# Mistra-UEA/Mistra

Hardware: AMD Instinct MI355X
Metric: chemistry-timesteps/sec (tot mechanism) (higher is better)
Workload: dtype f64; 1 GPU; tot mechanism, 100000 synthetic cells per GPU (100000 total), INTEGRATE_t(0,10 s), Ros3 rtol 1e-3; perturbed captured BTZ96 cloud states; cells_per_gpu=100000, failed_cells=0, parallelism=cells sharded over 1 GPU(s), no data-path collective

## Files before the change

### mistra_amd/build.py

```python
import os
import shutil
import subprocess
import sys

PKG = os.path.dirname(os.path.abspath(__file__))
CSRC = os.path.join(PKG, "csrc")
LIBDIR = os.path.join(PKG, "lib")
OBJDIR = os.path.join(PKG, "build")
LIB = os.path.join(LIBDIR, "libmistra_chem.so")

ARCH = "gfx950"
COMMON = ["-O3", "-std=c++17", "-fPIC", "-ffp-contract=off", "-fno-fast-math", "-Wall", "-Wno-unused-function"]
SOURCES = ["mech_tables.cpp", "schedule.cpp", "capi.cpp", "ros3_kernel.hip", "rates.hip", "pack.hip"]


def hipcc():
    for cand in (os.environ.get("HIPCC"), shutil.which("hipcc"), "/opt/rocm/bin/hipcc"):
        if cand and os.path.exists(cand):
            return cand
    raise RuntimeError("hipcc not found")


def _stale(target, deps):
    if not os.path.exists(target):
# ... 31 lines not shown
            print(" ".join(cmd))
        subprocess.run(cmd, check=True)
    return LIB


def ring_register_report(isa_path=None):
    import re
    import tempfile
    with tempfile.TemporaryDirectory() as tmp:
        if isa_path is None:
            isa_path = os.path.join(tmp, "ros3_kernel.s")
            cmd = [hipcc(), "--offload-arch=" + ARCH] + [f for f in COMMON if f != "-fPIC"] + \
                  ["-S", "--offload-device-only", os.path.join(CSRC, "ros3_kernel.hip"), "-o", isa_path]
            subprocess.run(cmd, check=True, stderr=subprocess.DEVNULL)
        lines = open(isa_path).read().split("\n")
    starts = [(i, l.split(":")[0]) for i, l in enumerate(lines) if re.match(r"^_ZN6mistra.*:", l)]
    starts.append((len(lines), "end"))
    report = {}
    ring_users = set()
    for (i, name), (j, _) in zip(starts, starts[1:]):
        in_asm, hi = False, 0
        for l in lines[i:j]:
            if "ASMSTART" in l:
                in_asm = True
            elif "ASMEND" in l:
                in_asm = False
            elif in_asm and re.search(r"global_load_dwordx4 v\[(64|192):\d+\], v\[\d+:\d+\], off", l):
                ring_users.add(name)
            elif "Folded Spill" in l or "Folded Reload" in l:
                pass
            elif not in_asm and not l.strip().startswith((";", ".")):
                for m in re.finditer(r"\bv(\d+)\b|\bv\[(\d+):(\d+)\]", l):
                    hi = max(hi, int(m.group(1) or m.group(3)))
        report[name] = hi
        low = re.search(r"(gsum_run|tail_solve|tail_solve_columns|scale_run)I.*Lb([01])E+[A-Z]", name)
        if low:
            limit = 64 if low.group(2) == "1" else 192
            if hi >= limit:
                raise RuntimeError("%s: the compiler allocates v%d, inside the look-ahead ring's register blocks (v%d..)" % (name, hi, limit))
        elif name in ring_users and "ros3_integrate_kernel" not in name:
            raise RuntimeError("%s issues look-ahead ring loads but is not covered by the register check" % name)
    report["__isa_text__"] = "\n".join(lines)
    return report


def isa_hazard_report(isa_text, sgpr_vmem_wait=5, dpp_wait=2, seen=None):
    import re
    hits = []
    seen = seen if seen is not None else {}
    for k in ("vmem_scalar_base", "dpp", "vmcnt", "functions"):
        seen.setdefault(k, 0)
    func, insts = None, []

    def regs(tok, kind):
        tok = tok.strip().lstrip("-").strip("|")
        m = re.match(r"^%s(\d+)$" % kind, tok)
        if m:
            return {int(m.group(1))}
        m = re.match(r"^%s\[(\d+):(\d+)\]$" % kind, tok)
        if m:
            return set(range(int(m.group(1)), int(m.group(2)) + 1))
        return set()

    def flush():
        if func is None:
            return
        seen["functions"] += 1
        depth = len({i["ops"][0] for i in insts if i["asm"] and i["op"].startswith(("global_load", "buffer_load")) and i["ops"]})
        for n, it in enumerate(insts):
            if not it["asm"]:
                continue
            op, ops = it["op"], it["ops"]
            if op.startswith(("global_", "buffer_", "scratch_", "flat_")):
                base = set()
                for o in ops:
                    if re.match(r"^s\[\d+:\d+\]$", o.strip()):
                        base |= regs(o, "s")
                if base:
                    seen["vmem_scalar_base"] += 1
                    waited, k = 0, n - 1
                    while k >= 0 and waited < sgpr_vmem_wait:
                        p = insts[k]
                        if p["op"] in ("v_readfirstlane_b32", "v_readlane_b32") and p["ops"] and regs(p["ops"][0], "s") & base:
                            hits.append("%s: line %d `%s` reads a scalar base written by `%s` %d wait state(s) earlier (needs %d)" %
                                        (func, it["line"], it["text"], p["text"], waited, sgpr_vmem_wait))
                            break
                        waited += p["wait"]
                        k -= 1
            if "_dpp" in op or re.search(r"\b(row_newbcast|row_shr|row_shl|row_ror|row_bcast|quad_perm|row_mirror|row_half_mirror|row_share|row_xmask):?", it["text"]):
                src0 = regs(ops[1], "v") if len(ops) > 1 else set()
                seen["dpp"] += 1
                waited, k = 0, n - 1
                while src0 and k >= 0 and waited < dpp_wait:
                    p = insts[k]
                    if p["op"].startswith("v_") and p["ops"] and regs(p["ops"][0], "v") & src0:
                        hits.append("%s: line %d `%s` DPP-reads a register written by `%s` %d wait state(s) earlier (needs %d)" %
                                    (func, it["line"], it["text"], p["text"], waited, dpp_wait))
                        break
                    waited += p["wait"]
                    k -= 1
            if op == "s_waitcnt" and depth:
                m = re.search(r"vmcnt\((\d+)\)", it["text"])
                seen["vmcnt"] += 1 if m else 0
                if m and int(m.group(1)) >= depth:
                    hits.append("%s: line %d `%s` waits for at most %s loads in flight, the function's asm loads fill only %d slots" %
                                (func, it["line"], it["text"], m.group(1), depth))

    in_asm = False
    for ln, raw in enumerate(isa_text.split("\n"), 1):
        if re.match(r"^[A-Za-z_.$][\w.$]*:", raw) and not raw.startswith(".L"):
            flush()
            func, insts, in_asm = raw.split(":")[0], [], False
            continue
        if "ASMSTART" in raw:
            in_asm = True
            continue
        if "ASMEND" in raw:
            in_asm = False
            continue
        t = raw.split(";")[0].strip()
        if not t or t.startswith(".") or t.endswith(":"):
            continue
        parts = t.split(None, 1)
        op = parts[0]
        ops = [o.strip() for o in re.split(r",(?![^\[]*\])", parts[1].split(" offset")[0])] if len(parts) > 1 else []
        ops = [o.split()[0] if o.split() else o for o in ops]
        wait = 1
        if op == "s_nop" and ops:
            wait = int(ops[0], 0) + 1
        insts.append({"op": op, "ops": ops, "asm": in_asm, "line": ln, "text": t, "wait": wait})
    flush()
    return hits


if __name__ == "__main__":
    print(build_lib(force="--force" in sys.argv, verbose=True))
```

### mistra_amd/csrc/capi.cpp

```cpp
#include "../../include/mistra_chem.h"

#include <dlfcn.h>
#include <hip/hip_runtime.h>

#include <algorithm>
#include <cstdio>
#include <cstdlib>
#include <cstring>
#include <mutex>
#include <string>
#include <thread>
#include <vector>

#include "kernel_args.hpp"
#include "mech_tables.hpp"
#include "pack.hpp"
#include "rates.hpp"
#include "ros3_kernel.hpp"
#include "schedule.hpp"

using namespace mistra;

namespace {

// ... 215 lines not shown
  int nrounds = 0;
  hipError_t upload(const VmProgram& P) {
    nrounds = P.nbarriers;
    hipError_t e;
    if ((e = wave_base.upload(P.wave_base)) != hipSuccess) return e;
    if ((e = blk_n.upload(P.blk_n)) != hipSuccess) return e;
    return recs.upload(P.recs);
  }
  VmDev dev() const { return VmDev{wave_base.p, blk_n.p, recs.p, nrounds}; }
  void release() { wave_base.release(); recs.release(); blk_n.release(); }
};

struct GsBufs {
  DevBuf<uint32_t> wave_base, recs;
  DevBuf<uint16_t> rows;
  hipError_t upload(const GsumProgram& P) {
    hipError_t e;
    if ((e = wave_base.upload(P.wave_base)) != hipSuccess) return e;
    if ((e = rows.upload(P.rows)) != hipSuccess) return e;
    return recs.upload(P.recs);
  }
  GsDev dev() const { return GsDev{wave_base.p, rows.p, recs.p}; }
  void release() { wave_base.release(); recs.release(); rows.release(); }
};


struct KernelBufs {
  int n_temps = 0, lu_scale_slots = 0;
  DevBuf<double> consts;
  DevBuf<uint64_t> fun_fac, jac_fac;
  DevBuf<uint16_t> jvs_pos, zero_pos, diag_pos, schur_cells;
  GsBufs vdot, jvs;
  VmBufs lu, solve_head_fwd, solve_head_bwd;
  DevBuf<uint32_t> tail_fwd, tail_bwd, lu_scale, dense_rows;
  int upload(const MechTables& t, const KernelSchedule& K) {
    n_temps = K.n_temps;
    lu_scale_slots = K.lu_scale.nslots;
    HIP_TRY(consts.upload(t.consts));
    HIP_TRY(fun_fac.upload(K.fun_fac));
    HIP_TRY(jac_fac.upload(K.jac_fac));
    HIP_TRY(jvs_pos.upload(K.jvs_pos));
    HIP_TRY(zero_pos.upload(K.zero_pos));
    HIP_TRY(diag_pos.upload(K.diag_pos));
    HIP_TRY(vdot.upload(K.vdot));
    HIP_TRY(jvs.upload(K.jvs));
    HIP_TRY(lu.upload(K.lu));
    HIP_TRY(solve_head_fwd.upload(K.solve_head_fwd));
    HIP_TRY(solve_head_bwd.upload(K.solve_head_bwd));
    HIP_TRY(tail_fwd.upload(K.tail.fwd));
    HIP_TRY(tail_bwd.upload(K.tail.bwd));
    HIP_TRY(lu_scale.upload(K.lu_scale.recs));
    HIP_TRY(dense_rows.upload(K.dense.row_info));
    HIP_TRY(schur_cells.upload(K.dense.schur_cells));
    return 0;
  }
  void release() {
    consts.release(); fun_fac.release(); jac_fac.release(); jvs_pos.release(); zero_pos.release(); diag_pos.release(); schur_cells.release();
    vdot.release(); jvs.release(); lu.release(); solve_head_fwd.release(); solve_head_bwd.release();
    tail_fwd.release(); tail_bwd.release(); lu_scale.release(); dense_rows.release();
  }
};

struct RatesBufs {
  bool ready = false;
  int nreact = 0, nenv = 0;
  DevBuf<double> consts;
  DevBuf<int32_t> offs, words, fslot;
  int upload(const RatesTable& T) {
    HIP_TRY(consts.upload(T.consts));
    HIP_TRY(offs.upload(T.offs));
    HIP_TRY(words.upload(T.words));
    HIP_TRY(fslot.upload(T.fslot));
    nreact = T.nreact; nenv = T.nenv;
    ready = true;
    return 0;
  }
  RatesDev dev() const { return RatesDev{consts.p, offs.p, words.p, fslot.p, nreact, nenv}; }
  void release() { consts.release(); offs.release(); words.release(); fslot.release(); ready = false; }
};

struct PackBufs {
  bool ready = false, maps_ready = false;
  PackTable tab;
  DevBuf<int32_t> pack, fix, unpack, slot_id, slot_first, terms, words, acc, envc, a_ptr, a_fac;
  DevBuf<int32_t> gas_m2k, gas_k2m, rad_m2k, rad_k2m;
  int j1 = 0, j5 = 0;
  int upload(const MechTables& t) {
    HIP_TRY(pack.upload(tab.pack)); HIP_TRY(fix.upload(tab.fix)); HIP_TRY(unpack.upload(tab.unpack));
    HIP_TRY(slot_id.upload(tab.slot_id)); HIP_TRY(slot_first.upload(tab.slot_first)); HIP_TRY(terms.upload(tab.terms));
    HIP_TRY(words.upload(tab.term_words)); HIP_TRY(acc.upload(tab.acc)); HIP_TRY(envc.upload(tab.envc));
    HIP_TRY(a_ptr.upload(t.a_ptr)); HIP_TRY(a_fac.upload(t.a_fac));
    ready = true;
// ... 293 lines not shown
    if (int rc = S.stc.upload()) return rc;
  }
  if (S.vmean.tab.load(base + ".vmean", &err)) {
    if (S.vmean.tab.nspec != nspec) return fail(name + ".vmean does not belong to this mechanism");
    if (int rc = S.vmean.upload()) return rc;
  }
  S.ready = true;
  return 0;
}

int launch(DeviceState& D, int mech, const KernelArgs& a, hipStream_t stream) {
  hipError_t e = hipErrorInvalidValue;
  if (mech == MISTRA_MECH_GAS) e = launch_ros3<GasTraits, kGasNT>(a, stream, &D.lds_configured[mech]);
  else if (mech == MISTRA_MECH_AER) e = launch_ros3<AerTraits, kAerNT>(a, stream, &D.lds_configured[mech]);
  else e = launch_ros3<TotTraits, kTotNT>(a, stream, &D.lds_configured[mech]);
  if (e != hipSuccess) return fail(std::string("kernel launch: ") + hipGetErrorString(e));
  return 0;
}

KernelArgs make_args(const MechState& S, int ncell, const double* var_in, const double* fix, const double* rconst, double tin,
                     double tout, double* var_out, int32_t* ierr, int32_t* stats, double* th) {
  const KernelBufs& k = S.k;
  KernelArgs a;
  a.var_in = var_in; a.fix = fix; a.rconst = rconst; a.var_out = var_out; a.ierr = ierr; a.stats = stats;
  a.texit_hexit = th; a.h_last = nullptr; a.hstart = nullptr; a.prof = nullptr; a.dump = nullptr; a.sing_rows = nullptr; a.n_temps = k.n_temps; a.max_steps = g_max_steps; a.tin = tin; a.tout = tout; a.ncell = ncell;
  a.consts = k.consts.p; a.fun_fac = k.fun_fac.p; a.jac_fac = k.jac_fac.p; a.jvs_pos = k.jvs_pos.p;
  a.zero_pos = k.zero_pos.p; a.diag_pos = k.diag_pos.p;
  a.vdot = k.vdot.dev(); a.jvs = k.jvs.dev(); a.lu = k.lu.dev();
#ifdef MISTRA_DIAG_ENV
  if (const char* cut = std::getenv("MISTRA_DIAG_LU_ROUNDS"))
    a.lu.nrounds = std::max(1, std::min(a.lu.nrounds, std::atoi(cut)));
#endif
  a.solve_head_fwd = k.solve_head_fwd.dev(); a.solve_head_bwd = k.solve_head_bwd.dev();
  a.tail = TailDev{k.tail_fwd.p, k.tail_bwd.p};
  a.lu_scale = ScaleDev{k.lu_scale.p, k.lu_scale_slots, k.lu_scale_slots + VM_LOOKAHEAD_ROWS};
  a.dense = DenseDev{k.dense_rows.p, k.schur_cells.p};
  return a;
}

PackDev pack_dev(const MechState& S) { return S.pack.dev(S.tab.nreact, S.k.consts.p); }

int check_call(int mech, int ncell) {
  if (mech < 0 || mech > 2) return fail("unknown mechanism id");
  if (ncell < 0) return fail("negative cell count");
  if (!g_inited || g_devs.empty() || !g_devs[0].mech[mech].ready) return fail("mistra_chem_init has not been called (or failed)");
  return 0;
}

int require(const MechState& S, int mech, unsigned need) {
  const std::string m = kMechName[mech];
  if ((need & kNeedPackTable) && !S.pack.ready) return fail("no hand-over table for the " + m + " mechanism");
  if ((need & kNeedMaps) && !S.pack.maps_ready) return fail("mistra_chem_set_species_maps has not been called for the " + m + " mechanism");
  if ((need & kNeedRates) && !S.rates.ready) return fail("no device rate table for the " + m + " mechanism");
  if ((need & kNeedKmt) && !S.kmt.ready) return fail("the " + m + " mechanism has no mass-transfer routine (fast_k_mt_a: aer, fast_k_mt_t: tot)");
  if ((need & kNeedLiq) && !S.liq.ready)
    return fail("the " + m + " mechanism has no liquid-phase routines (henry_a / equil_co_a: aer, henry_t / equil_co_t: tot)");
  if ((need & kNeedStc) && !S.stc.ready) return fail("the " + m + " mechanism has no st_coeff routine (st_coeff_a: aer, st_coeff_t: tot)");
  if ((need & kNeedVmean) && !S.vmean.ready) return fail("the " + m + " mechanism has no v_mean routine (v_mean_a: aer, v_mean_t: tot)");
  return 0;
}

struct Slot {
  DeviceState* D = nullptr;
  MechState* S = nullptr;
};

int on_device(int mech, int ncell, const void* p, const char* what, unsigned need, Slot* t) {
// ... 971 lines not shown
```

### mistra_amd/csrc/kernel_args.hpp

```cpp
#pragma once
#include <cstdint>

namespace mistra {

constexpr int kProfSlots = 16;
constexpr int kVmSweepUpdPerRec = 3;

struct VmDev {
  const uint32_t* wave_base;
  const uint16_t* blk_n;
  const uint32_t* recs;
  int nrounds;
};

struct GsDev {
  const uint32_t* wave_base;
  const uint16_t* rows;
  const uint32_t* recs;
};

struct ScaleDev {
  const uint32_t* recs;
  int nslots;
  int wave_slots;
};

struct TailDev {
  const uint32_t* fwd;
  const uint32_t* bwd;
};

struct DenseDev {
  const uint32_t* row_info;
  const uint16_t* schur_cells;
};

struct KernelArgs {
  const double* var_in;
  const double* fix;
  const double* rconst;
  double* var_out;
  int32_t* ierr;
  int32_t* stats;
  double* texit_hexit;
  const double* hstart;
  double* h_last;
  int32_t* sing_rows;
  double* dump;
  unsigned long long* prof;
  double tin, tout;
  int32_t ncell;
  int32_t n_temps;
  int32_t max_steps;
  const double* consts;
  const uint64_t* fun_fac;
  const uint64_t* jac_fac;
  const uint16_t* jvs_pos;
  const uint16_t* zero_pos;
  const uint16_t* diag_pos;
  GsDev vdot, jvs;
  VmDev lu, solve_head_fwd, solve_head_bwd;
  ScaleDev lu_scale;
// ... 6 lines not shown
```

### mistra_amd/csrc/ros3_kernel.hip

```cpp
#include <hip/hip_runtime.h>

#include <cstdint>
#include <type_traits>

#include "kernel_args.hpp"
#include "ros3_kernel.hpp"

namespace mistra {

namespace {

constexpr uint16_t kPosDiag = 0x8000, kPosNone = 0xFFFF;
constexpr int kRingSlots = 8;

typedef uint32_t u32x4 __attribute__((ext_vector_type(4)));
typedef float f32x4 __attribute__((ext_vector_type(4)));

template <class T>
using gptr = const T __attribute__((address_space(1)))*;
template <class T>
using gptr_mut = T __attribute__((address_space(1)))*;
template <class T>
__device__ __forceinline__ gptr<T> G_(const T* p) { return (gptr<T>)p; }
template <class T>
// ... 305 lines not shown
               : [x] "+v"(x) : [xb] "v"(xb), MISTRA_TAIL_COPS)
#define MISTRA_UPDATE_BWD(ROWMASK)                                                                                             \
  asm volatile("s_nop 1\n\t"                                                                                                   \
               MISTRA_UPD_STEP(15, ROWMASK) MISTRA_UPD_STEP(14, ROWMASK) MISTRA_UPD_STEP(13, ROWMASK) MISTRA_UPD_STEP(12, ROWMASK) \
               MISTRA_UPD_STEP(11, ROWMASK) MISTRA_UPD_STEP(10, ROWMASK) MISTRA_UPD_STEP(9, ROWMASK) MISTRA_UPD_STEP(8, ROWMASK)   \
               MISTRA_UPD_STEP(7, ROWMASK) MISTRA_UPD_STEP(6, ROWMASK) MISTRA_UPD_STEP(5, ROWMASK) MISTRA_UPD_STEP(4, ROWMASK)     \
               MISTRA_UPD_STEP(3, ROWMASK) MISTRA_UPD_STEP(2, ROWMASK) MISTRA_UPD_STEP(1, ROWMASK)                                 \
               "v_fmac_f64_dpp %[x], -%[xb], %[c0] row_newbcast:0 row_mask:" ROWMASK " bank_mask:0xf"                           \
               : [x] "+v"(x) : [xb] "v"(xb), MISTRA_TAIL_COPS)

template <int ROW, bool BACKWARD>
__device__ __forceinline__ void tail_diag(double& x, const double (&c)[16]) {
  if constexpr (!BACKWARD) {
    if constexpr (ROW == 0) MISTRA_DIAG_FWD("0x1");
    else if constexpr (ROW == 1) MISTRA_DIAG_FWD("0x2");
    else if constexpr (ROW == 2) MISTRA_DIAG_FWD("0x4");
    else MISTRA_DIAG_FWD("0x8");
  } else {
    if constexpr (ROW == 0) MISTRA_DIAG_BWD("0x1");
    else if constexpr (ROW == 1) MISTRA_DIAG_BWD("0x2");
    else if constexpr (ROW == 2) MISTRA_DIAG_BWD("0x4");
    else MISTRA_DIAG_BWD("0x8");
  }
}
template <int MASK, bool BACKWARD>
__device__ __forceinline__ void tail_update(double& x, const double xb, const double (&c)[16]) {
  static_assert(MASK >= 1 && MASK <= 15, "row mask");
#define MISTRA_UPD_CASE(M, S) else if constexpr (MASK == M) { if constexpr (BACKWARD) MISTRA_UPDATE_BWD(S); else MISTRA_UPDATE_FWD(S); }
  if constexpr (MASK == 15) { if constexpr (BACKWARD) MISTRA_UPDATE_BWD("0xf"); else MISTRA_UPDATE_FWD("0xf"); }
  MISTRA_UPD_CASE(14, "0xe") MISTRA_UPD_CASE(12, "0xc") MISTRA_UPD_CASE(8, "0x8") MISTRA_UPD_CASE(1, "0x1") MISTRA_UPD_CASE(3, "0x3") MISTRA_UPD_CASE(7, "0x7")
  else static_assert(MASK == 15, "row mask not instantiated");
#undef MISTRA_UPD_CASE
}
#undef MISTRA_DIAG_STEP
#undef MISTRA_DIAG_FWD
#undef MISTRA_DIAG_BWD
#undef MISTRA_UPD_STEP
#undef MISTRA_UPDATE_FWD
#undef MISTRA_UPDATE_BWD
#undef MISTRA_TAIL_COPS

template <int R, int J, bool BACKWARD, bool LAST, class NEXT>
__device__ __forceinline__ void tail_block(double (&xr)[R], double (&c)[16], const uint32_t (&ad)[16], NEXT&& next) {
  constexpr int REG = J / 4, ROW = J % 4;
  constexpr int OTHER = BACKWARD ? 0 : R - 1;
  constexpr bool HAS_OTHER = !LAST && R == 2 && REG != OTHER;
  double d[16];
  if constexpr (HAS_OTHER) {
#pragma unroll
    for (int j = 0; j < 16; j++) d[j] = lds_ld(ad[BACKWARD ? 15 - j : j]);
  }
  double x = xr[REG];
  tail_diag<ROW, BACKWARD>(x, c);
  if constexpr (!LAST) {
    const double xb = lane_row_to_all<ROW>(x);
    constexpr int same = BACKWARD ? (1 << ROW) - 1 : (0xF << (ROW + 1)) & 0xF;
    if constexpr (same != 0) tail_update<same, BACKWARD>(x, xb, c);
    xr[REG] = x;
    if constexpr (HAS_OTHER) {
      double y = xr[OTHER];
      asm volatile("" : "+v"(y), "+v"(d[0]), "+v"(d[15]));
      next();
      tail_update<15, BACKWARD>(y, xb, d);
      xr[OTHER] = y;
    } else {
      next();
    }
  } else {
    xr[REG] = x;
    next();
  }
}

template <int R, int FWD_BLOCK0, bool LOW>
__device__ __attribute__((noinline)) void tail_solve(const TailDev T, uint32_t xb, uint32_t rb, int lane) {
  constexpr int NB = 4 * R;
  constexpr int NF = NB - FWD_BLOCK0;
  constexpr int NS = NF + NB;
  static_assert(FWD_BLOCK0 >= 0 && FWD_BLOCK0 <= NB && NS <= 16, "first forward block");
  double x[R], rd[R];
#pragma unroll
  for (int r = 0; r < R; r++) {
    x[r] = lds_ld(xb + 8 * (r * 64 + lane));
    rd[r] = lds_ld(rb + 8 * (r * 64 + lane));
  }
  const uint64_t tf = ring_base(T.fwd + FWD_BLOCK0 * 4 * 64 * 4).b0, tb = ring_base(T.bwd).b0;
  const uint32_t voff = 16u * (uint32_t)lane;
  uint32_t three = 3;
  asm volatile("" : "+v"(three));
#define MISTRA_TAIL_LOADS(S, K0)                                                                                          \
  {                                                                                                                      \
    const uint64_t base = (S) < NF ? tf + (uint64_t)(S) * 4096u : tb + (uint64_t)((S) - NF) * 4096u;                     \
    vm_ring_load_at<LOW, K0, 0>(base, voff); vm_ring_load_at<LOW, K0 + 1, 1024>(base, voff);                             \
    vm_ring_load_at<LOW, K0 + 2, 2048>(base, voff); vm_ring_load_at<LOW, K0 + 3, 3072>(base, voff);                      \
  }
  asm volatile("s_waitcnt vmcnt(0)" : : : "memory");
  MISTRA_TAIL_LOADS(0, 0) MISTRA_TAIL_LOADS(1, 4)
  double c[16];
  uint32_t ad[16];
#define MISTRA_TAIL_GATHER(S)                                                                                             \
  if constexpr ((S) < NS) {                                                                                              \
    constexpr int K0 = ((S) & 1) * 4;                                                                                    \
    constexpr bool BW = (S) >= NF;                                                                                       \
    constexpr int J = BW ? (NB - 1 - ((S) - NF) + NB) % NB : (FWD_BLOCK0 + (S)) % NB;                                    \
    constexpr int REG = J / 4, OTHER = BW ? 0 : R - 1;                                                                   \
    constexpr bool LAST = BW ? (S) == NS - 1 : FWD_BLOCK0 + (S) == NB - 1;                                               \
    constexpr bool HAS_OTHER = !LAST && R == 2 && REG != OTHER;                                                          \
    constexpr bool LO = REG == 0 || (HAS_OTHER && OTHER == 0), HI = REG == 1 || (HAS_OTHER && OTHER == 1);               \
    uint32_t ac[16];                                                                                                     \
    uint32_t* const alo = REG == 0 ? ac : ad;                                                                            \
    uint32_t* const ahi = REG == 1 ? ac : ad;                                                                            \
    vm_ring_take_cells<LOW, K0, 7, LO, HI>(alo, ahi, three);         vm_ring_take_cells<LOW, K0 + 1, 6, LO, HI>(alo + 4, ahi + 4, three);   \
    vm_ring_take_cells<LOW, K0 + 2, 5, LO, HI>(alo + 8, ahi + 8, three); vm_ring_take_cells<LOW, K0 + 3, 4, LO, HI>(alo + 12, ahi + 12, three); \
    MISTRA_TAIL_LOADS((S) + 2, K0)                                                                                       \
    _Pragma("unroll") for (int j = 0; j < 16; j++) c[j] = lds_ld(ac[BW ? 15 - j : j]);                                   \
  }
#define MISTRA_TAIL_STEP(S)                                                                                               \
  if constexpr ((S) < NS) {                                                                                              \
    if constexpr ((S) == NF) {                                                                                           \
      _Pragma("unroll") for (int r = 0; r < R; r++) x[r] = x[r] * rd[r];                                                 \
    }                                                                                                                    \
    auto next = [&]() { MISTRA_TAIL_GATHER((S) + 1) };                                                                   \
    if constexpr ((S) < NF) tail_block<R, (FWD_BLOCK0 + (S)) % NB, false, FWD_BLOCK0 + (S) == NB - 1>(x, c, ad, next);   \
    else tail_block<R, (NB - 1 - ((S) - NF) + NB) % NB, true, (S) == NS - 1>(x, c, ad, next);                            \
  }
  MISTRA_TAIL_GATHER(0)
  MISTRA_TAIL_STEP(0) MISTRA_TAIL_STEP(1) MISTRA_TAIL_STEP(2) MISTRA_TAIL_STEP(3) MISTRA_TAIL_STEP(4) MISTRA_TAIL_STEP(5) MISTRA_TAIL_STEP(6) MISTRA_TAIL_STEP(7)
  MISTRA_TAIL_STEP(8) MISTRA_TAIL_STEP(9) MISTRA_TAIL_STEP(10) MISTRA_TAIL_STEP(11) MISTRA_TAIL_STEP(12) MISTRA_TAIL_STEP(13) MISTRA_TAIL_STEP(14) MISTRA_TAIL_STEP(15)
#undef MISTRA_TAIL_STEP
#undef MISTRA_TAIL_GATHER
#undef MISTRA_TAIL_LOADS
  asm volatile("s_waitcnt vmcnt(0)" : : : "memory");
#pragma unroll
  for (int r = 0; r < R; r++) lds_st(xb + 8 * (r * 64 + lane), x[r]);
}

__device__ __forceinline__ double readlane_f64(double v, int l) {
  const uint64_t u = __builtin_bit_cast(uint64_t, v);
  const uint32_t lo = (uint32_t)__builtin_amdgcn_readlane((int)(uint32_t)u, l);
  const uint32_t hi = (uint32_t)__builtin_amdgcn_readlane((int)(uint32_t)(u >> 32), l);
  return __builtin_bit_cast(double, (uint64_t)lo | ((uint64_t)hi << 32));
}

template <int R, int FWD_FROM, bool LOW>
__device__ __attribute__((noinline)) void tail_solve_columns(const TailDev T, uint32_t xb, uint32_t rb, int lane) {
  constexpr int FWD_END = R;
  constexpr bool FORWARD = FWD_FROM < FWD_END;
  constexpr uint32_t mb = 0;
  double x[R], rd[R];
  const uint32_t voff = 16u * (uint32_t)lane;
  static_assert(R == 1 || R == 2, "one or two 64-row registers");
  uint32_t three = 3;
  asm volatile("" : "+v"(three));
#pragma unroll
  for (int r = 0; r < R; r++) x[r] = lds_ld(xb + 8 * (r * 64 + lane));
#define MISTRA_TAIL_OPERANDS(BUF, K, PENDING)                                           \
  {                                                                                     \
    uint32_t alo[4], ahi[4];                                                            \
    vm_ring_take_cells<LOW, K, PENDING, true, R == 2>(alo, ahi, three);                 \
    _Pragma("unroll") for (int c = 0; c < 4; c++) {                                     \
      BUF[c][0] = lds_ld(mb + alo[c]);                                                  \
      if constexpr (R == 2) BUF[c][1] = lds_ld(mb + ahi[c]);                            \
    }                                                                                   \
  }
// ... 1014 lines not shown
```

### mistra_amd/csrc/schedule.cpp

```cpp
#include "schedule.hpp"

#include <algorithm>
#include <cassert>
#include <cstdio>
#include <cstdlib>
#include <cstring>
#include <iterator>
#include <map>
#include <numeric>
#include <stdexcept>

namespace mistra {

namespace {

inline const char* diag_env(const char* name) {
#ifdef MISTRA_DIAG_ENV
  return std::getenv(name);
#else
  (void)name;
  return nullptr;
#endif
}

// ... 692 lines not shown
    }
    rows.push_back(std::move(E));
  }
  if (temps_used) *temps_used = used;
  parts.insert(parts.end(), std::make_move_iterator(rows.begin()), std::make_move_iterator(rows.end()));
  return parts;
}

TailSolve build_tail_solve(const MechTables& m, const VmLayout& lay, int regs) {
  TailSolve T;
  const int n = m.nvar, zero_slot = lay.zero();
  T.regs = regs > 0 ? regs : n > 128 + 64 ? 2 : 1;
  T.m = 64 * T.regs;
  if (T.m > n) throw std::invalid_argument("mechanism smaller than one wave");
  T.h = n - T.m;
  if (zero_slot > 0xFFFF) throw std::invalid_argument("tail tables need 16-bit Ghimj slots");
  const uint32_t z = (uint32_t)zero_slot;
  T.fwd.assign(((size_t)T.m / 4 + VM_LOOKAHEAD_ROWS) * 256, z | (z << 16));
  T.bwd.assign(((size_t)T.m / 4 + VM_LOOKAHEAD_ROWS) * 256, z | (z << 16));
  auto put = [&](std::vector<uint32_t>& tab, int group_pos, int lane, int r, int slot) {
    uint32_t& w = tab[((size_t)(group_pos / 4) * 64 + lane) * 4 + group_pos % 4];
    w = r == 0 ? ((w & 0xFFFF0000u) | (uint32_t)slot) : ((w & 0x0000FFFFu) | ((uint32_t)slot << 16));
  };
  for (int ti = 0; ti < T.m; ti++) {
    const int i = T.h + ti, lane = ti % 64, r = ti / 64;
    for (int p = m.crow[i]; p < m.crow[i + 1]; p++) {
      const int c = m.icol[p];
      if (c < T.h || c == i) continue;
      const int q = c - T.h;
      if (c < i) put(T.fwd, q, lane, r, p);
      else put(T.bwd, T.m - 1 - q, lane, r, p);
    }
  }
  return T;
}

DenseTail build_dense_tail(const MechTables& m, const VmLayout& lay, int nd, int kb) {
  DenseTail D;
  const int n = m.nvar;
  if (nd != 64) throw std::invalid_argument("the dense tail block is 64 rows (8 waves x 2 tiles of 16x16)");
  D.nd = nd;
  D.h = n - nd;
  D.kb = kb;
  D.jm = D.h - 4 * kb;
  if (D.jm < 0 || kb < 0) throw std::invalid_argument("more Schur steps than pivots");
  if (D.info_rows() > DenseTail::kInfoRowsMax) throw std::invalid_argument("too many Schur steps for the LDS row table");
  D.row_info.assign((size_t)DenseTail::kInfoRowsMax * 4, 0u);
  auto describe_range = [&](int g, int row, int c0, int c1) {
    int first = -1, seen = 0;
    uint64_t absent = 0;
    for (int c = c0; c < c1; c++) {
      int slot = -1;
      for (int p = m.crow[row]; p < m.crow[row + 1]; p++)
        if (m.icol[p] == c) slot = p;
      if (slot < 0) { absent |= 1ull << (c - c0); continue; }
      if (first < 0) first = slot;
      if (slot != first + seen) throw std::logic_error("dense tail: a row's slots inside a column range are not contiguous");
      seen++;
    }
    for (int c = c1 - c0; c < 64; c++) absent |= 1ull << c;
    D.row_info[(size_t)g * 4] = (uint32_t)std::max(first, 0);
    D.row_info[(size_t)g * 4 + 1] = (uint32_t)absent;
    D.row_info[(size_t)g * 4 + 2] = (uint32_t)(absent >> 32);
  };
  for (int i = 0; i < nd; i++) {
    describe_range(i, D.h + i, D.h, n);
// ... 250 lines not shown
```

### mistra_amd/csrc/schedule.hpp

```cpp
#pragma once
#include <cstdint>
#include <string>
#include <utility>
#include <vector>

#include "kernel_args.hpp"
#include "mech_tables.hpp"

namespace mistra {

constexpr uint32_t VM_D1_RCP = 1u;
constexpr uint32_t VM_D1_CONT = 2u;
constexpr uint32_t VM_ROW_EOR = 1u << 24;
constexpr uint32_t VM_ROW_NULL = 1u << 25;
constexpr uint32_t VM_ROW_AUX = 1u << 26;
constexpr uint32_t VM_ROW_LOCAL = 1u << 27;
constexpr int VM_ROW_EOR_BIT = 24, VM_ROW_NULL_BIT = 25, VM_ROW_AUX_BIT = 26, VM_ROW_LOCAL_BIT = 27;
constexpr uint32_t VM_AUX_MASK = 0x00FFFFF8u;
constexpr int VM_REC_WORDS = 8;
inline size_t vm_rec_index(size_t row, int lane, int k) { return row * 512 + (k < 4 ? 0 : 256) + (size_t)lane * 4 + (size_t)(k & 3); }
constexpr int VM_UPD_PER_REC = 2;
constexpr int VM_SWEEP_UPD_PER_REC = kVmSweepUpdPerRec;
constexpr int VM_LOOKAHEAD_ROWS = 16;

// ... 19 lines not shown

struct VmEntry {
  int tgt = 0;
  int mulr = -1;
  int rcp = -1;
  int phase = 0;
  bool keep_order = true;
  std::vector<VmUpd> upd;
};

struct VmProgram {
  int nt = 0, nw = 0, nrounds = 0, zero_slot = 0;
  int nbarriers = 0;
  int upd_per_rec = VM_UPD_PER_REC;
  std::vector<uint32_t> wave_base;
  std::vector<uint16_t> blk_n;
  std::vector<uint32_t> recs;
  int64_t n_updates = 0, n_items = 0, n_records = 0, wave_rows = 0, crit_rows = 0;
  int64_t lds_cycles = 0;
};

struct GsumProgram {
  int nt = 0, nw = 0, nq = 0;
  std::vector<uint32_t> wave_base;
  std::vector<uint16_t> rows;
  std::vector<uint32_t> recs;
  int64_t n_terms = 0, wave_rows = 0;
};

struct TailSolve {
  int m = 0, h = 0, regs = 0;
  std::vector<uint32_t> fwd;
  std::vector<uint32_t> bwd;
};

struct ScaleProgram {
  int nt = 0, nw = 0, nslots = 0;
  std::vector<uint32_t> recs;
  int64_t n_pairs = 0;
};

struct DenseTail {
  int nd = 0, h = 0, jm = 0, kb = 0;
  std::vector<uint32_t> row_info;
  std::vector<uint16_t> schur_cells;
  size_t schur_w(int I, int k, int lane) const { return ((size_t)I * kb + k) * 64 + lane; }
  size_t schur_u(int half, int k, int t, int lane) const { return (size_t)4 * kb * 64 + (((size_t)half * kb + k) * 2 + t) * 64 + lane; }
  static constexpr int kInfoRowsMax = 192;
  int info_rows() const { return 128 + 4 * kb; }
  int cell(int g, int c) const {
    const uint64_t mask = (uint64_t)row_info[(size_t)g * 4 + 1] | ((uint64_t)row_info[(size_t)g * 4 + 2] << 32);
    if ((mask >> c) & 1) return -1;
    return (int)row_info[(size_t)g * 4] + c - __builtin_popcountll(mask & ((1ull << c) - 1));
  }
};

struct DenseConfig { int nd, kb; };
#ifndef MISTRA_TOT_DENSE
#define MISTRA_TOT_DENSE 1
#endif
inline DenseConfig dense_config(const MechTables& m) { return m.nvar == 417 && MISTRA_TOT_DENSE ? DenseConfig{64, 14} : DenseConfig{0, 0}; }

struct KernelSchedule {
  int nt = 0, nw = 0;
  int spt = 0;
  int rpt = 0;
// ... 41 lines not shown
```

Measured before the change: 25740 chemistry-timesteps/s.

## Precompute tail-solve LDS addresses and interleave gathers with DPP diagonal steps

The tail triangular solve used to unpack packed 16-bit cell indices from the look-ahead ring at run time and then issue separate LDS loads. Per-register byte-address tables are now built on the host, so the ring loads deliver ready LDS addresses. The next block's ds_read_b64 gathers are interleaved in inline assembly with the current block's DPP fmac diagonal and update steps, overlapping LDS latency with the dependent chain. In exchange there are more uploaded tables, a new group/ring indexing scheme, more hand-written asm register constraints, and extended build-time register and hazard checks.

```diff
diff --git a/mistra_amd/build.py b/mistra_amd/build.py
--- a/mistra_amd/build.py
+++ b/mistra_amd/build.py
@@ -87,6 +87,12 @@
             elif not in_asm and not l.strip().startswith((";", ".")):
                 for m in re.finditer(r"\bv(\d+)\b|\bv\[(\d+):(\d+)\]", l):
                     hi = max(hi, int(m.group(1) or m.group(3)))
+            elif in_asm and not l.strip().startswith((";", ".")):
+                t = l.split(";")[0].strip().split(None, 1)
+                if len(t) == 2 and t[0].startswith("v_") or len(t) == 2 and t[0].startswith("ds_read"):
+                    m = re.match(r"\s*(?:v(\d+)\b|v\[(\d+):(\d+)\])", t[1])
+                    if m:
+                        hi = max(hi, int(m.group(1) or m.group(3)))
         report[name] = hi
         low = re.search(r"(gsum_run|tail_solve|tail_solve_columns|scale_run)I.*Lb([01])E+[A-Z]", name)
         if low:
@@ -121,7 +127,11 @@
         if func is None:
             return
         seen["functions"] += 1
-        depth = len({i["ops"][0] for i in insts if i["asm"] and i["op"].startswith(("global_load", "buffer_load")) and i["ops"]})
+        loads = [i for i in insts if i["asm"] and i["op"].startswith(("global_load", "buffer_load")) and i["ops"]]
+        depth = len({i["ops"][0] for i in loads})
+        block_depth = {}
+        for i in loads:
+            block_depth.setdefault(i["block"], set()).add(i["ops"][0])
         for n, it in enumerate(insts):
             if not it["asm"]:
                 continue
@@ -157,18 +167,20 @@
             if op == "s_waitcnt" and depth:
                 m = re.search(r"vmcnt\((\d+)\)", it["text"])
                 seen["vmcnt"] += 1 if m else 0
-                if m and int(m.group(1)) >= depth:
-                    hits.append("%s: line %d `%s` waits for at most %s loads in flight, the function's asm loads fill only %d slots" %
-                                (func, it["line"], it["text"], m.group(1), depth))
-
-    in_asm = False
+                own = len(block_depth.get(it["block"], ()))
+                if m and int(m.group(1)) >= (own or depth):
+                    hits.append("%s: line %d `%s` waits for at most %s loads in flight, %s fill only %d slots" %
+                                (func, it["line"], it["text"], m.group(1), "its asm block's loads" if own else "the function's asm loads",
+                                 own or depth))
+
+    in_asm, block = False, 0
     for ln, raw in enumerate(isa_text.split("\n"), 1):
         if re.match(r"^[A-Za-z_.$][\w.$]*:", raw) and not raw.startswith(".L"):
             flush()
             func, insts, in_asm = raw.split(":")[0], [], False
             continue
         if "ASMSTART" in raw:
-            in_asm = True
+            in_asm, block = True, block + 1
             continue
         if "ASMEND" in raw:
             in_asm = False
@@ -183,7 +195,7 @@
         wait = 1
         if op == "s_nop" and ops:
             wait = int(ops[0], 0) + 1
-        insts.append({"op": op, "ops": ops, "asm": in_asm, "line": ln, "text": t, "wait": wait})
+        insts.append({"op": op, "ops": ops, "asm": in_asm, "block": block if in_asm else 0, "line": ln, "text": t, "wait": wait})
     flush()
     return hits
 
diff --git a/mistra_amd/csrc/capi.cpp b/mistra_amd/csrc/capi.cpp
--- a/mistra_amd/csrc/capi.cpp
+++ b/mistra_amd/csrc/capi.cpp
@@ -271,7 +271,7 @@
   DevBuf<uint16_t> jvs_pos, zero_pos, diag_pos, schur_cells;
   GsBufs vdot, jvs;
   VmBufs lu, solve_head_fwd, solve_head_bwd;
-  DevBuf<uint32_t> tail_fwd, tail_bwd, lu_scale, dense_rows;
+  DevBuf<uint32_t> tail_fwd, tail_bwd, tail_fwd_addr[2], tail_bwd_addr[2], lu_scale, dense_rows;
   int upload(const MechTables& t, const KernelSchedule& K) {
     n_temps = K.n_temps;
     lu_scale_slots = K.lu_scale.nslots;
@@ -288,6 +288,10 @@
     HIP_TRY(solve_head_bwd.upload(K.solve_head_bwd));
     HIP_TRY(tail_fwd.upload(K.tail.fwd));
     HIP_TRY(tail_bwd.upload(K.tail.bwd));
+    for (int r = 0; r < 2; r++) {
+      HIP_TRY(tail_fwd_addr[r].upload(K.tail.fwd_addr[r]));
+      HIP_TRY(tail_bwd_addr[r].upload(K.tail.bwd_addr[r]));
+    }
     HIP_TRY(lu_scale.upload(K.lu_scale.recs));
     HIP_TRY(dense_rows.upload(K.dense.row_info));
     HIP_TRY(schur_cells.upload(K.dense.schur_cells));
@@ -297,6 +301,7 @@
     consts.release(); fun_fac.release(); jac_fac.release(); jvs_pos.release(); zero_pos.release(); diag_pos.release(); schur_cells.release();
     vdot.release(); jvs.release(); lu.release(); solve_head_fwd.release(); solve_head_bwd.release();
     tail_fwd.release(); tail_bwd.release(); lu_scale.release(); dense_rows.release();
+    for (int r = 0; r < 2; r++) { tail_fwd_addr[r].release(); tail_bwd_addr[r].release(); }
   }
 };
 
@@ -656,7 +661,7 @@
     a.lu.nrounds = std::max(1, std::min(a.lu.nrounds, std::atoi(cut)));
 #endif
   a.solve_head_fwd = k.solve_head_fwd.dev(); a.solve_head_bwd = k.solve_head_bwd.dev();
-  a.tail = TailDev{k.tail_fwd.p, k.tail_bwd.p};
+  a.tail = TailDev{k.tail_fwd.p, k.tail_bwd.p, {k.tail_fwd_addr[0].p, k.tail_fwd_addr[1].p}, {k.tail_bwd_addr[0].p, k.tail_bwd_addr[1].p}};
   a.lu_scale = ScaleDev{k.lu_scale.p, k.lu_scale_slots, k.lu_scale_slots + VM_LOOKAHEAD_ROWS};
   a.dense = DenseDev{k.dense_rows.p, k.schur_cells.p};
   return a;
diff --git a/mistra_amd/csrc/kernel_args.hpp b/mistra_amd/csrc/kernel_args.hpp
--- a/mistra_amd/csrc/kernel_args.hpp
+++ b/mistra_amd/csrc/kernel_args.hpp
@@ -28,6 +28,8 @@
 struct TailDev {
   const uint32_t* fwd;
   const uint32_t* bwd;
+  const uint32_t* fwd_addr[2];
+  const uint32_t* bwd_addr[2];
 };
 
 struct DenseDev {
diff --git a/mistra_amd/csrc/ros3_kernel.hip b/mistra_amd/csrc/ros3_kernel.hip
--- a/mistra_amd/csrc/ros3_kernel.hip
+++ b/mistra_amd/csrc/ros3_kernel.hip
@@ -361,6 +361,107 @@
   else static_assert(MASK == 15, "row mask not instantiated");
 #undef MISTRA_UPD_CASE
 }
+#define MISTRA_TAIL_GOPS                                                                                                          \
+  [g0] "=&v"(g[0]), [g1] "=&v"(g[1]), [g2] "=&v"(g[2]), [g3] "=&v"(g[3]), [g4] "=&v"(g[4]), [g5] "=&v"(g[5]), [g6] "=&v"(g[6]),           \
+      [g7] "=&v"(g[7]), [g8] "=&v"(g[8]), [g9] "=&v"(g[9]), [g10] "=&v"(g[10]), [g11] "=&v"(g[11]), [g12] "=&v"(g[12]),                   \
+      [g13] "=&v"(g[13]), [g14] "=&v"(g[14]), [g15] "=&v"(g[15])
+#define MISTRA_RING_HALF_HI0 192, 193, 194, 195, 196, 197, 198, 199, 208, 209, 210, 211, 212, 213, 214, 215
+#define MISTRA_RING_HALF_HI1 224, 225, 226, 227, 228, 229, 230, 231, 240, 241, 242, 243, 244, 245, 246, 247
+#define MISTRA_RING_HALF_LO0 64, 65, 66, 67, 68, 69, 70, 71, 80, 81, 82, 83, 84, 85, 86, 87
+#define MISTRA_RING_HALF_LO1 96, 97, 98, 99, 100, 101, 102, 103, 112, 113, 114, 115, 116, 117, 118, 119
+#define MISTRA_APPLY(M, ...) M(__VA_ARGS__)
+#define MISTRA_ON_RING_HALF(M, ...)                                                                                            \
+  if constexpr (LOW && H == 0) MISTRA_APPLY(M, __VA_ARGS__, MISTRA_RING_HALF_LO0);                                            \
+  else if constexpr (LOW) MISTRA_APPLY(M, __VA_ARGS__, MISTRA_RING_HALF_LO1);                                                 \
+  else if constexpr (H == 0) MISTRA_APPLY(M, __VA_ARGS__, MISTRA_RING_HALF_HI0);                                              \
+  else MISTRA_APPLY(M, __VA_ARGS__, MISTRA_RING_HALF_HI1);
+#define MISTRA_G2(A, RA, B, RB) "ds_read_b64 %[g" #A "], v" #RA "\n\tds_read_b64 %[g" #B "], v" #RB "\n\t"
+#define MISTRA_G16(r0, r1, r2, r3, r4, r5, r6, r7, r8, r9, r10, r11, r12, r13, r14, r15)                                        \
+  MISTRA_G2(0, r0, 1, r1) MISTRA_G2(2, r2, 3, r3) MISTRA_G2(4, r4, 5, r5) MISTRA_G2(6, r6, 7, r7) MISTRA_G2(8, r8, 9, r9)       \
+      MISTRA_G2(10, r10, 11, r11) MISTRA_G2(12, r12, 13, r13) MISTRA_G2(14, r14, 15, r15)
+#define MISTRA_DSTEP(J, RM) "v_fmac_f64_dpp %[x], -%[x], %[c" #J "] row_newbcast:" #J " row_mask:" RM " bank_mask:0xf\n\t"
+#define MISTRA_NSTEP(J, RM) "s_nop 1\n\t" MISTRA_DSTEP(J, RM)
+#define MISTRA_DIAG_G_FWD(RM, r0, r1, r2, r3, r4, r5, r6, r7, r8, r9, r10, r11, r12, r13, r14, r15)                               \
+  asm volatile("s_waitcnt vmcnt(4)\n\t"                                                                                       \
+               MISTRA_G2(0, r0, 1, r1) MISTRA_DSTEP(0, RM) MISTRA_G2(2, r2, 3, r3) MISTRA_DSTEP(1, RM)                        \
+               MISTRA_G2(4, r4, 5, r5) MISTRA_DSTEP(2, RM) MISTRA_G2(6, r6, 7, r7) MISTRA_DSTEP(3, RM)                        \
+               MISTRA_G2(8, r8, 9, r9) MISTRA_DSTEP(4, RM) MISTRA_G2(10, r10, 11, r11) MISTRA_DSTEP(5, RM)                    \
+               MISTRA_G2(12, r12, 13, r13) MISTRA_DSTEP(6, RM) MISTRA_G2(14, r14, 15, r15) MISTRA_DSTEP(7, RM)                \
+               MISTRA_NSTEP(8, RM) MISTRA_NSTEP(9, RM) MISTRA_NSTEP(10, RM) MISTRA_NSTEP(11, RM) MISTRA_NSTEP(12, RM)         \
+               MISTRA_NSTEP(13, RM) MISTRA_NSTEP(14, RM) "s_waitcnt lgkmcnt(0)"              \
+               : [x] "+v"(x), MISTRA_TAIL_GOPS : MISTRA_TAIL_COPS : "memory")
+#define MISTRA_DIAG_G_BWD(RM, r0, r1, r2, r3, r4, r5, r6, r7, r8, r9, r10, r11, r12, r13, r14, r15)                               \
+  asm volatile("s_waitcnt vmcnt(4)\n\t"                                                                                       \
+               MISTRA_G2(0, r0, 1, r1) MISTRA_DSTEP(15, RM) MISTRA_G2(2, r2, 3, r3) MISTRA_DSTEP(14, RM)                      \
+               MISTRA_G2(4, r4, 5, r5) MISTRA_DSTEP(13, RM) MISTRA_G2(6, r6, 7, r7) MISTRA_DSTEP(12, RM)                      \
+               MISTRA_G2(8, r8, 9, r9) MISTRA_DSTEP(11, RM) MISTRA_G2(10, r10, 11, r11) MISTRA_DSTEP(10, RM)                  \
+               MISTRA_G2(12, r12, 13, r13) MISTRA_DSTEP(9, RM) MISTRA_G2(14, r14, 15, r15) MISTRA_DSTEP(8, RM)                \
+               MISTRA_NSTEP(7, RM) MISTRA_NSTEP(6, RM) MISTRA_NSTEP(5, RM) MISTRA_NSTEP(4, RM) MISTRA_NSTEP(3, RM)            \
+               MISTRA_NSTEP(2, RM) MISTRA_NSTEP(1, RM) "s_waitcnt lgkmcnt(0)"                 \
+               : [x] "+v"(x), MISTRA_TAIL_GOPS : MISTRA_TAIL_COPS : "memory")
+#define MISTRA_USTEP(J) "v_fmac_f64_dpp %[x], -%[xb], %[c" #J "] row_newbcast:" #J " row_mask:0xf bank_mask:0xf\n\t"
+#define MISTRA_UPDATE_G_FWD(UNUSED, r0, r1, r2, r3, r4, r5, r6, r7, r8, r9, r10, r11, r12, r13, r14, r15)                                 \
+  asm volatile("s_waitcnt vmcnt(4)\n\t"                                                                                       \
+               MISTRA_G2(0, r0, 1, r1) MISTRA_USTEP(0) MISTRA_G2(2, r2, 3, r3) MISTRA_USTEP(1)                                \
+               MISTRA_G2(4, r4, 5, r5) MISTRA_USTEP(2) MISTRA_G2(6, r6, 7, r7) MISTRA_USTEP(3)                                \
+               MISTRA_G2(8, r8, 9, r9) MISTRA_USTEP(4) MISTRA_G2(10, r10, 11, r11) MISTRA_USTEP(5)                            \
+               MISTRA_G2(12, r12, 13, r13) MISTRA_USTEP(6) MISTRA_G2(14, r14, 15, r15) MISTRA_USTEP(7)                        \
+               MISTRA_USTEP(8) MISTRA_USTEP(9) MISTRA_USTEP(10) MISTRA_USTEP(11) MISTRA_USTEP(12) MISTRA_USTEP(13)            \
+               MISTRA_USTEP(14) MISTRA_USTEP(15) "s_waitcnt lgkmcnt(0)"                                                       \
+               : [x] "+v"(x), MISTRA_TAIL_GOPS : [xb] "v"(xb), MISTRA_TAIL_COPS : "memory")
+#define MISTRA_UPDATE_G_BWD(UNUSED, r0, r1, r2, r3, r4, r5, r6, r7, r8, r9, r10, r11, r12, r13, r14, r15)                                 \
+  asm volatile("s_waitcnt vmcnt(4)\n\t"                                                                                       \
+               MISTRA_G2(0, r0, 1, r1) MISTRA_USTEP(15) MISTRA_G2(2, r2, 3, r3) MISTRA_USTEP(14)                              \
+               MISTRA_G2(4, r4, 5, r5) MISTRA_USTEP(13) MISTRA_G2(6, r6, 7, r7) MISTRA_USTEP(12)                              \
+               MISTRA_G2(8, r8, 9, r9) MISTRA_USTEP(11) MISTRA_G2(10, r10, 11, r11) MISTRA_USTEP(10)                          \
+               MISTRA_G2(12, r12, 13, r13) MISTRA_USTEP(9) MISTRA_G2(14, r14, 15, r15) MISTRA_USTEP(8)                        \
+               MISTRA_USTEP(7) MISTRA_USTEP(6) MISTRA_USTEP(5) MISTRA_USTEP(4) MISTRA_USTEP(3) MISTRA_USTEP(2)                \
+               MISTRA_USTEP(1) MISTRA_USTEP(0) "s_waitcnt lgkmcnt(0)"                                                         \
+               : [x] "+v"(x), MISTRA_TAIL_GOPS : [xb] "v"(xb), MISTRA_TAIL_COPS : "memory")
+#define MISTRA_GATHER_ONLY(UNUSED, r0, r1, r2, r3, r4, r5, r6, r7, r8, r9, r10, r11, r12, r13, r14, r15)                                  \
+  asm volatile("s_waitcnt vmcnt(4)\n\t" MISTRA_G16(r0, r1, r2, r3, r4, r5, r6, r7, r8, r9, r10, r11, r12, r13, r14, r15)       \
+               "s_waitcnt lgkmcnt(0)" : MISTRA_TAIL_GOPS : : "memory")
+
+template <bool LOW, int H, int ROW, bool BACKWARD>
+__device__ __forceinline__ void tail_diag_gather(double& x, const double (&c)[16], double (&g)[16]) {
+  if constexpr (!BACKWARD) {
+    if constexpr (ROW == 0) { MISTRA_ON_RING_HALF(MISTRA_DIAG_G_FWD, "0x1") }
+    else if constexpr (ROW == 1) { MISTRA_ON_RING_HALF(MISTRA_DIAG_G_FWD, "0x2") }
+    else if constexpr (ROW == 2) { MISTRA_ON_RING_HALF(MISTRA_DIAG_G_FWD, "0x4") }
+    else { MISTRA_ON_RING_HALF(MISTRA_DIAG_G_FWD, "0x8") }
+  } else {
+    if constexpr (ROW == 0) { MISTRA_ON_RING_HALF(MISTRA_DIAG_G_BWD, "0x1") }
+    else if constexpr (ROW == 1) { MISTRA_ON_RING_HALF(MISTRA_DIAG_G_BWD, "0x2") }
+    else if constexpr (ROW == 2) { MISTRA_ON_RING_HALF(MISTRA_DIAG_G_BWD, "0x4") }
+    else { MISTRA_ON_RING_HALF(MISTRA_DIAG_G_BWD, "0x8") }
+  }
+}
+template <bool LOW, int H, bool BACKWARD>
+__device__ __forceinline__ void tail_update_gather(double& x, const double xb, const double (&c)[16], double (&g)[16]) {
+  if constexpr (BACKWARD) { MISTRA_ON_RING_HALF(MISTRA_UPDATE_G_BWD, 0) }
+  else { MISTRA_ON_RING_HALF(MISTRA_UPDATE_G_FWD, 0) }
+}
+template <bool LOW, int H>
+__device__ __forceinline__ void tail_gather(double (&g)[16]) {
+  MISTRA_ON_RING_HALF(MISTRA_GATHER_ONLY, 0)
+}
+#undef MISTRA_TAIL_GOPS
+#undef MISTRA_RING_HALF_HI0
+#undef MISTRA_RING_HALF_HI1
+#undef MISTRA_RING_HALF_LO0
+#undef MISTRA_RING_HALF_LO1
+#undef MISTRA_APPLY
+#undef MISTRA_ON_RING_HALF
+#undef MISTRA_G2
+#undef MISTRA_G16
+#undef MISTRA_DSTEP
+#undef MISTRA_NSTEP
+#undef MISTRA_DIAG_G_FWD
+#undef MISTRA_DIAG_G_BWD
+#undef MISTRA_USTEP
+#undef MISTRA_UPDATE_G_FWD
+#undef MISTRA_UPDATE_G_BWD
+#undef MISTRA_GATHER_ONLY
 #undef MISTRA_DIAG_STEP
 #undef MISTRA_DIAG_FWD
 #undef MISTRA_DIAG_BWD
@@ -369,18 +470,50 @@
 #undef MISTRA_UPDATE_BWD
 #undef MISTRA_TAIL_COPS
 
-template <int R, int J, bool BACKWARD, bool LAST, class NEXT>
-__device__ __forceinline__ void tail_block(double (&xr)[R], double (&c)[16], const uint32_t (&ad)[16], NEXT&& next) {
-  constexpr int REG = J / 4, ROW = J % 4;
-  constexpr int OTHER = BACKWARD ? 0 : R - 1;
-  constexpr bool HAS_OTHER = !LAST && R == 2 && REG != OTHER;
-  double d[16];
+template <int R, int FWD_BLOCK0>
+struct TailStream {
+  static constexpr int NB = 4 * R;
+  static constexpr int NF = NB - FWD_BLOCK0;
+  static constexpr int NS = NF + NB;
+  static constexpr bool bw(int s) { return s >= NF; }
+  static constexpr int col_block(int s) { return bw(s) ? NB - 1 - (s - NF) : FWD_BLOCK0 + s; }
+  static constexpr bool last(int s) { return bw(s) ? s == NS - 1 : FWD_BLOCK0 + s == NB - 1; }
+  static constexpr int reg(int s) { return col_block(s) / 4; }
+  static constexpr int other(int s) { return bw(s) ? 0 : R - 1; }
+  static constexpr bool has_other(int s) { return !last(s) && R == 2 && reg(s) != other(s); }
+  static constexpr int own_group(int s) {
+    int g = 0;
+    for (int i = 0; i < s && i < NS; i++) g += has_other(i) ? 2 : 1;
+    return g;
+  }
+  static constexpr int NG = own_group(NS);
+  static constexpr int group_block(int g) {
+    int s = 0;
+    while (s + 1 < NS && own_group(s + 1) <= g) s++;
+    return s;
+  }
+  static constexpr int group_reg(int g) { return g == own_group(group_block(g)) ? reg(group_block(g)) : other(group_block(g)); }
+};
+
+template <class TS, int S, bool LOW, int R, class LOAD>
+__device__ __forceinline__ void tail_block(double (&xr)[R], double (&c)[16], LOAD&& load) {
+  constexpr int J = TS::col_block(S), REG = J / 4, ROW = J % 4, OTHER = TS::other(S);
+  constexpr bool BACKWARD = TS::bw(S), LAST = TS::last(S), HAS_OTHER = TS::has_other(S), NEXT = S + 1 < TS::NS;
+  constexpr int GO = TS::own_group(S) + 1, GN = TS::own_group(S + 1);
+  constexpr bool DIAG_NEXT = !HAS_OTHER && NEXT && !LOW;
+  double x = xr[REG];
+  double g[16], d[16];
   if constexpr (HAS_OTHER) {
-#pragma unroll
-    for (int j = 0; j < 16; j++) d[j] = lds_ld(ad[BACKWARD ? 15 - j : j]);
-  }
-  double x = xr[REG];
-  tail_diag<ROW, BACKWARD>(x, c);
+    tail_diag_gather<LOW, GO & 1, ROW, BACKWARD>(x, c, g);
+    load(std::integral_constant<int, GO + 2>());
+#pragma unroll
+    for (int j = 0; j < 16; j++) d[j] = g[BACKWARD ? 15 - j : j];
+  } else if constexpr (DIAG_NEXT) {
+    tail_diag_gather<LOW, GN & 1, ROW, BACKWARD>(x, c, g);
+    load(std::integral_constant<int, GN + 2>());
+  } else {
+    tail_diag<ROW, BACKWARD>(x, c);
+  }
   if constexpr (!LAST) {
     const double xb = lane_row_to_all<ROW>(x);
     constexpr int same = BACKWARD ? (1 << ROW) - 1 : (0xF << (ROW + 1)) & 0xF;
@@ -388,77 +521,76 @@
     xr[REG] = x;
     if constexpr (HAS_OTHER) {
       double y = xr[OTHER];
-      asm volatile("" : "+v"(y), "+v"(d[0]), "+v"(d[15]));
-      next();
-      tail_update<15, BACKWARD>(y, xb, d);
+      tail_update_gather<LOW, GN & 1, BACKWARD>(y, xb, d, g);
       xr[OTHER] = y;
-    } else {
-      next();
+      load(std::integral_constant<int, GN + 2>());
+    } else if constexpr (!DIAG_NEXT) {
+      tail_gather<LOW, GN & 1>(g);
+      load(std::integral_constant<int, GN + 2>());
     }
   } else {
     xr[REG] = x;
-    next();
+    if constexpr (NEXT && !DIAG_NEXT) {
+      tail_gather<LOW, GN & 1>(g);
+      load(std::integral_constant<int, GN + 2>());
+    }
+  }
+  if constexpr (NEXT) {
+#pragma unroll
+    for (int j = 0; j < 16; j++) c[j] = g[TS::bw(S + 1) ? 15 - j : j];
   }
 }
 
 template <int R, int FWD_BLOCK0, bool LOW>
 __device__ __attribute__((noinline)) void tail_solve(const TailDev T, uint32_t xb, uint32_t rb, int lane) {
-  constexpr int NB = 4 * R;
-  constexpr int NF = NB - FWD_BLOCK0;
-  constexpr int NS = NF + NB;
-  static_assert(FWD_BLOCK0 >= 0 && FWD_BLOCK0 <= NB && NS <= 16, "first forward block");
+  using TS = TailStream<R, FWD_BLOCK0>;
+  static_assert(FWD_BLOCK0 >= 0 && FWD_BLOCK0 <= TS::NB && TS::NS <= 16, "first forward block");
   double x[R], rd[R];
 #pragma unroll
   for (int r = 0; r < R; r++) {
     x[r] = lds_ld(xb + 8 * (r * 64 + lane));
     rd[r] = lds_ld(rb + 8 * (r * 64 + lane));
   }
-  const uint64_t tf = ring_base(T.fwd + FWD_BLOCK0 * 4 * 64 * 4).b0, tb = ring_base(T.bwd).b0;
+  uint64_t tf[R], tb[R];
+#pragma unroll
+  for (int r = 0; r < R; r++) {
+    tf[r] = ring_base(T.fwd_addr[r]).b0;
+    tb[r] = ring_base(T.bwd_addr[r]).b0;
+  }
   const uint32_t voff = 16u * (uint32_t)lane;
-  uint32_t three = 3;
-  asm volatile("" : "+v"(three));
-#define MISTRA_TAIL_LOADS(S, K0)                                                                                          \
-  {                                                                                                                      \
-    const uint64_t base = (S) < NF ? tf + (uint64_t)(S) * 4096u : tb + (uint64_t)((S) - NF) * 4096u;                     \
-    vm_ring_load_at<LOW, K0, 0>(base, voff); vm_ring_load_at<LOW, K0 + 1, 1024>(base, voff);                             \
-    vm_ring_load_at<LOW, K0 + 2, 2048>(base, voff); vm_ring_load_at<LOW, K0 + 3, 3072>(base, voff);                      \
-  }
+  auto load = [&](auto group) {
+    constexpr int G = decltype(group)::value, K0 = 4 * (G & 1);
+    uint64_t base;
+    if constexpr (G < TS::NG) {
+      constexpr int s = TS::group_block(G), r = TS::group_reg(G);
+      base = TS::bw(s) ? tb[r] + (uint64_t)(s - TS::NF) * 4096u : tf[r] + (uint64_t)TS::col_block(s) * 4096u;
+    } else {
+      base = tb[0] + (uint64_t)(TS::NB + G - TS::NG) * 4096u;
+    }
+    vm_ring_load_at<LOW, K0, 0>(base, voff); vm_ring_load_at<LOW, K0 + 1, 1024>(base, voff);
+    vm_ring_load_at<LOW, K0 + 2, 2048>(base, voff); vm_ring_load_at<LOW, K0 + 3, 3072>(base, voff);
+  };
   asm volatile("s_waitcnt vmcnt(0)" : : : "memory");
-  MISTRA_TAIL_LOADS(0, 0) MISTRA_TAIL_LOADS(1, 4)
+  load(std::integral_constant<int, 0>());
+  load(std::integral_constant<int, 1>());
   double c[16];
-  uint32_t ad[16];
-#define MISTRA_TAIL_GATHER(S)                                                                                             \
-  if constexpr ((S) < NS) {                                                                                              \
-    constexpr int K0 = ((S) & 1) * 4;                                                                                    \
-    constexpr bool BW = (S) >= NF;                                                                                       \
-    constexpr int J = BW ? (NB - 1 - ((S) - NF) + NB) % NB : (FWD_BLOCK0 + (S)) % NB;                                    \
-    constexpr int REG = J / 4, OTHER = BW ? 0 : R - 1;                                                                   \
-    constexpr bool LAST = BW ? (S) == NS - 1 : FWD_BLOCK0 + (S) == NB - 1;                                               \
-    constexpr bool HAS_OTHER = !LAST && R == 2 && REG != OTHER;                                                          \
-    constexpr bool LO = REG == 0 || (HAS_OTHER && OTHER == 0), HI = REG == 1 || (HAS_OTHER && OTHER == 1);               \
-    uint32_t ac[16];                                                                                                     \
-    uint32_t* const alo = REG == 0 ? ac : ad;                                                                            \
-    uint32_t* const ahi = REG == 1 ? ac : ad;                                                                            \
-    vm_ring_take_cells<LOW, K0, 7, LO, HI>(alo, ahi, three);         vm_ring_take_cells<LOW, K0 + 1, 6, LO, HI>(alo + 4, ahi + 4, three);   \
-    vm_ring_take_cells<LOW, K0 + 2, 5, LO, HI>(alo + 8, ahi + 8, three); vm_ring_take_cells<LOW, K0 + 3, 4, LO, HI>(alo + 12, ahi + 12, three); \
-    MISTRA_TAIL_LOADS((S) + 2, K0)                                                                                       \
-    _Pragma("unroll") for (int j = 0; j < 16; j++) c[j] = lds_ld(ac[BW ? 15 - j : j]);                                   \
+  {
+    double g[16];
+    tail_gather<LOW, 0>(g);
+    load(std::integral_constant<int, 2>());
+#pragma unroll
+    for (int j = 0; j < 16; j++) c[j] = g[TS::bw(0) ? 15 - j : j];
   }
 #define MISTRA_TAIL_STEP(S)                                                                                               \
-  if constexpr ((S) < NS) {                                                                                              \
-    if constexpr ((S) == NF) {                                                                                           \
+  if constexpr ((S) < TS::NS) {                                                                                          \
+    if constexpr ((S) == TS::NF) {                                                                                       \
       _Pragma("unroll") for (int r = 0; r < R; r++) x[r] = x[r] * rd[r];                                                 \
     }                                                                                                                    \
-    auto next = [&]() { MISTRA_TAIL_GATHER((S) + 1) };                                                                   \
-    if constexpr ((S) < NF) tail_block<R, (FWD_BLOCK0 + (S)) % NB, false, FWD_BLOCK0 + (S) == NB - 1>(x, c, ad, next);   \
-    else tail_block<R, (NB - 1 - ((S) - NF) + NB) % NB, true, (S) == NS - 1>(x, c, ad, next);                            \
-  }
-  MISTRA_TAIL_GATHER(0)
+    tail_block<TS, (S), LOW>(x, c, load);                                                                                \
+  }
   MISTRA_TAIL_STEP(0) MISTRA_TAIL_STEP(1) MISTRA_TAIL_STEP(2) MISTRA_TAIL_STEP(3) MISTRA_TAIL_STEP(4) MISTRA_TAIL_STEP(5) MISTRA_TAIL_STEP(6) MISTRA_TAIL_STEP(7)
   MISTRA_TAIL_STEP(8) MISTRA_TAIL_STEP(9) MISTRA_TAIL_STEP(10) MISTRA_TAIL_STEP(11) MISTRA_TAIL_STEP(12) MISTRA_TAIL_STEP(13) MISTRA_TAIL_STEP(14) MISTRA_TAIL_STEP(15)
 #undef MISTRA_TAIL_STEP
-#undef MISTRA_TAIL_GATHER
-#undef MISTRA_TAIL_LOADS
   asm volatile("s_waitcnt vmcnt(0)" : : : "memory");
 #pragma unroll
   for (int r = 0; r < R; r++) lds_st(xb + 8 * (r * 64 + lane), x[r]);
diff --git a/mistra_amd/csrc/schedule.cpp b/mistra_amd/csrc/schedule.cpp
--- a/mistra_amd/csrc/schedule.cpp
+++ b/mistra_amd/csrc/schedule.cpp
@@ -748,6 +748,15 @@
       else put(T.bwd, T.m - 1 - q, lane, r, p);
     }
   }
+  auto addresses = [](const std::vector<uint32_t>& tab, int r) {
+    std::vector<uint32_t> a(tab.size());
+    for (size_t k = 0; k < tab.size(); k++) a[k] = 8u * ((tab[k] >> (16 * r)) & 0xFFFFu);
+    return a;
+  };
+  for (int r = 0; r < T.regs; r++) {
+    T.fwd_addr[r] = addresses(T.fwd, r);
+    T.bwd_addr[r] = addresses(T.bwd, r);
+  }
   return T;
 }
 
diff --git a/mistra_amd/csrc/schedule.hpp b/mistra_amd/csrc/schedule.hpp
--- a/mistra_amd/csrc/schedule.hpp
+++ b/mistra_amd/csrc/schedule.hpp
@@ -75,6 +75,7 @@
   int m = 0, h = 0, regs = 0;
   std::vector<uint32_t> fwd;
   std::vector<uint32_t> bwd;
+  std::vector<uint32_t> fwd_addr[2], bwd_addr[2];
 };
 
 struct ScaleProgram {
```

New measurement: 26530 chemistry-timesteps/s (median of 6 runs). 1.03x the previous value.
